# alexandre01/deepsvg

Measured on NVIDIA H100. Metric: icons/sec train-step (fwd+loss+bwd) hierarchical_ordered, higher is better.
Workload: dtype bf16

## Files before the change

### deepsvg_b200/csrc/attention_mma.cu

```cuda
#include "../../include/dsvg_b200.h"
#include "common.cuh"

namespace dsvg {
extern unsigned long long g_launches;

constexpr int kRow = 40;
constexpr int kTile = 32 * kRow;

struct MmaAttnArgs {
  const bf16* qkv;
  const uint8_t* valid;
  bf16* out;
  const bf16* dout;
  bf16* dqkv;
  int nseq, L, H;
  float scale;
  Dropout drop;
  int causal;
};

__device__ __forceinline__ void mma_bf16(float (&c)[4], const uint32_t (&a)[4], uint32_t b0, uint32_t b1) {
  asm volatile(
      "mma.sync.aligned.m16n8k16.row.col.f32.bf16.bf16.f32 {%0,%1,%2,%3}, {%4,%5,%6,%7}, {%8,%9}, {%0,%1,%2,%3};\n"
      : "+f"(c[0]), "+f"(c[1]), "+f"(c[2]), "+f"(c[3])
      : "r"(a[0]), "r"(a[1]), "r"(a[2]), "r"(a[3]), "r"(b0), "r"(b1));
}
__device__ __forceinline__ void ldsm_x4(uint32_t (&r)[4], uint32_t addr) {
  asm volatile("ldmatrix.sync.aligned.m8n8.x4.shared.b16 {%0,%1,%2,%3}, [%4];\n"
               : "=r"(r[0]), "=r"(r[1]), "=r"(r[2]), "=r"(r[3]) : "r"(addr));
}
__device__ __forceinline__ void ldsm_x4_t(uint32_t (&r)[4], uint32_t addr) {
  asm volatile("ldmatrix.sync.aligned.m8n8.x4.trans.shared.b16 {%0,%1,%2,%3}, [%4];\n"
               : "=r"(r[0]), "=r"(r[1]), "=r"(r[2]), "=r"(r[3]) : "r"(addr));
}
__device__ __forceinline__ uint32_t pack_bf16(float lo, float hi) {
  __nv_bfloat162 v = __floats2bfloat162_rn(lo, hi);
  return *reinterpret_cast<uint32_t*>(&v);
}
__device__ __forceinline__ uint32_t smem_addr(const void* p) { return uint32_t(__cvta_generic_to_shared(p)); }

__device__ __forceinline__ void load_a(uint32_t (&a)[4], uint32_t tile, int mt, int ks, int lane) {
  const int m = lane >> 3, r = lane & 7;
  ldsm_x4(a, tile + ((16 * mt + (m & 1) * 8 + r) * kRow + 16 * ks + (m >> 1) * 8) * 2);
}
__device__ __forceinline__ void load_a_t(uint32_t (&a)[4], uint32_t tile, int mt, int ks, int lane) {
  const int m = lane >> 3, r = lane & 7;
  ldsm_x4_t(a, tile + ((16 * ks + (m >> 1) * 8 + r) * kRow + 16 * mt + (m & 1) * 8) * 2);
}
__device__ __forceinline__ void load_b_nk(uint32_t (&b)[4], uint32_t tile, int np, int ks, int lane) {
  const int m = lane >> 3, r = lane & 7;
  ldsm_x4(b, tile + ((16 * np + (m >> 1) * 8 + r) * kRow + 16 * ks + (m & 1) * 8) * 2);
}
__device__ __forceinline__ void load_b_kn(uint32_t (&b)[4], uint32_t tile, int np, int ks, int lane) {
  const int m = lane >> 3, r = lane & 7;
  ldsm_x4_t(b, tile + ((16 * ks + (m & 1) * 8 + r) * kRow + 16 * np + (m >> 1) * 8) * 2);
}

__device__ __forceinline__ void stage_tile(bf16* dst, const bf16* src, int ld, int L, int lane) {
#pragma unroll
  for (int it = 0; it < 4; ++it) {
    const int chunk = lane + 32 * it, row = chunk >> 2, part = chunk & 3;
    uint4 v = make_uint4(0, 0, 0, 0);
    if (row < L) v = *reinterpret_cast<const uint4*>(src + size_t(row) * ld + part * 8);
    *reinterpret_cast<uint4*>(dst + row * kRow + part * 8) = v;
  }
}

__device__ __forceinline__ void softmax_rows(float (&s)[2][4][4], uint32_t key_mask, int t, int g = 0, int causal = 0) {
#pragma unroll
  for (int mt = 0; mt < 2; ++mt)
#pragma unroll
    for (int hrow = 0; hrow < 2; ++hrow) {
      float m = -INFINITY;
      const int i = 16 * mt + g + 8 * hrow;
      const uint32_t km = causal ? (key_mask & (0xFFFFFFFFu >> (31 - i))) : key_mask;
#pragma unroll
      for (int nt = 0; nt < 4; ++nt)
#pragma unroll
        for (int e = 0; e < 2; ++e) {
          const int j = 8 * nt + 2 * t + e;
          float& x = s[mt][nt][2 * hrow + e];
          if (!((km >> j) & 1u)) x = -INFINITY;
          m = fmaxf(m, x);
        }
      m = fmaxf(m, __shfl_xor_sync(0xffffffffu, m, 1));
      m = fmaxf(m, __shfl_xor_sync(0xffffffffu, m, 2));
      float sum = 0.f;
#pragma unroll
      for (int nt = 0; nt < 4; ++nt)
#pragma unroll
        for (int e = 0; e < 2; ++e) {
          float& x = s[mt][nt][2 * hrow + e];
          x = __expf(x - m);
          sum += x;
        }
      sum += __shfl_xor_sync(0xffffffffu, sum, 1);
      sum += __shfl_xor_sync(0xffffffffu, sum, 2);
      const float inv = 1.f / sum;
#pragma unroll
      for (int nt = 0; nt < 4; ++nt)
#pragma unroll
        for (int e = 0; e < 2; ++e) s[mt][nt][2 * hrow + e] *= inv;
    }
}

__device__ __forceinline__ void dropout_tile(float (&mult)[2][4][4], const Dropout& d, unsigned long long pair, int g,
                                             int t) {
#pragma unroll
  for (int mt = 0; mt < 2; ++mt)
#pragma unroll
    for (int hrow = 0; hrow < 2; ++hrow) {
      const int i = 16 * mt + g + 8 * hrow;
      const unsigned long long quad = ((pair * 32 + i) * 4 + t) * 2;
      const uint32_t hk = drop_hikey(d, quad), q0 = uint32_t(quad);
#pragma unroll
      for (int hq = 0; hq < 2; ++hq) {
        const uint32_t s1 = drop_stage1(q0 + hq, hk);
        const uint32_t a = drop_fin_a(s1), b = drop_fin_b(s1);
        mult[mt][2 * hq][2 * hrow] = drop_keep_lo(a, d.thr16) ? d.scale : 0.f;
        mult[mt][2 * hq][2 * hrow + 1] = drop_keep_hi(a, d.thr16) ? d.scale : 0.f;
        mult[mt][2 * hq + 1][2 * hrow] = drop_keep_lo(b, d.thr16) ? d.scale : 0.f;
        mult[mt][2 * hq + 1][2 * hrow + 1] = drop_keep_hi(b, d.thr16) ? d.scale : 0.f;
      }
    }
}

__device__ __forceinline__ uint32_t key_mask_of(const uint8_t* valid, size_t row0, int L, int lane) {
  bool ok = lane < L;
  if (ok && valid != nullptr) ok = valid[row0 + lane] != 0;
  return __ballot_sync(0xffffffffu, ok);
}

__device__ __forceinline__ void qk_scores(float (&s)[2][4][4], uint32_t q_tile, uint32_t k_tile, int lane) {
#pragma unroll
  for (int mt = 0; mt < 2; ++mt)
#pragma unroll
    for (int nt = 0; nt < 4; ++nt)
#pragma unroll
      for (int e = 0; e < 4; ++e) s[mt][nt][e] = 0.f;
#pragma unroll
  for (int ks = 0; ks < 2; ++ks) {
    uint32_t a[2][4];
    load_a(a[0], q_tile, 0, ks, lane);
    load_a(a[1], q_tile, 1, ks, lane);
#pragma unroll
    for (int np = 0; np < 2; ++np) {
      uint32_t b[4];
      load_b_nk(b, k_tile, np, ks, lane);
#pragma unroll
      for (int mt = 0; mt < 2; ++mt) {
        mma_bf16(s[mt][2 * np], a[mt], b[0], b[1]);
        mma_bf16(s[mt][2 * np + 1], a[mt], b[2], b[3]);
      }
    }
  }
}

__device__ __forceinline__ void c_to_a(uint32_t (&a)[4], const float (&c)[2][4][4], int mt, int ks) {
  a[0] = pack_bf16(c[mt][2 * ks][0], c[mt][2 * ks][1]);
  a[1] = pack_bf16(c[mt][2 * ks][2], c[mt][2 * ks][3]);
  a[2] = pack_bf16(c[mt][2 * ks + 1][0], c[mt][2 * ks + 1][1]);
  a[3] = pack_bf16(c[mt][2 * ks + 1][2], c[mt][2 * ks + 1][3]);
}
__device__ __forceinline__ void mul_regs_kn(float (&o)[2][4][4], const float (&p)[2][4][4], uint32_t y_tile, int lane) {
#pragma unroll
  for (int mt = 0; mt < 2; ++mt)
#pragma unroll
    for (int nt = 0; nt < 4; ++nt)
#pragma unroll
      for (int e = 0; e < 4; ++e) o[mt][nt][e] = 0.f;
#pragma unroll
  for (int ks = 0; ks < 2; ++ks) {
    uint32_t a[2][4];
    c_to_a(a[0], p, 0, ks);
    c_to_a(a[1], p, 1, ks);
#pragma unroll
    for (int np = 0; np < 2; ++np) {
      uint32_t b[4];
      load_b_kn(b, y_tile, np, ks, lane);
#pragma unroll
      for (int mt = 0; mt < 2; ++mt) {
        mma_bf16(o[mt][2 * np], a[mt], b[0], b[1]);
        mma_bf16(o[mt][2 * np + 1], a[mt], b[2], b[3]);
      }
    }
  }
}
__device__ __forceinline__ void mul_t_kn(float (&o)[2][4][4], uint32_t z_tile, uint32_t y_tile, int lane) {
#pragma unroll
  for (int mt = 0; mt < 2; ++mt)
#pragma unroll
    for (int nt = 0; nt < 4; ++nt)
#pragma unroll
      for (int e = 0; e < 4; ++e) o[mt][nt][e] = 0.f;
#pragma unroll
  for (int ks = 0; ks < 2; ++ks) {
    uint32_t a[2][4];
    load_a_t(a[0], z_tile, 0, ks, lane);
    load_a_t(a[1], z_tile, 1, ks, lane);
#pragma unroll
    for (int np = 0; np < 2; ++np) {
      uint32_t b[4];
      load_b_kn(b, y_tile, np, ks, lane);
#pragma unroll
      for (int mt = 0; mt < 2; ++mt) {
        mma_bf16(o[mt][2 * np], a[mt], b[0], b[1]);
        mma_bf16(o[mt][2 * np + 1], a[mt], b[2], b[3]);
      }
    }
  }
}
__device__ __forceinline__ void store_c_global(bf16* dst, int ld, int L, const float (&c)[2][4][4], float mul, int g,
                                               int t) {
#pragma unroll
  for (int mt = 0; mt < 2; ++mt)
#pragma unroll
    for (int hrow = 0; hrow < 2; ++hrow) {
      const int i = 16 * mt + g + 8 * hrow;
      if (i < L) {
#pragma unroll
        for (int nt = 0; nt < 4; ++nt)
          *reinterpret_cast<uint32_t*>(dst + size_t(i) * ld + 8 * nt + 2 * t) =
              pack_bf16(c[mt][nt][2 * hrow] * mul, c[mt][nt][2 * hrow + 1] * mul);
      }
    }
}
__device__ __forceinline__ void store_c_smem(bf16* tile, const float (&c)[2][4][4], int g, int t) {
#pragma unroll
  for (int mt = 0; mt < 2; ++mt)
#pragma unroll
    for (int hrow = 0; hrow < 2; ++hrow) {
      const int i = 16 * mt + g + 8 * hrow;
#pragma unroll
      for (int nt = 0; nt < 4; ++nt)
        *reinterpret_cast<uint32_t*>(tile + i * kRow + 8 * nt + 2 * t) = pack_bf16(c[mt][nt][2 * hrow], c[mt][nt][2 * hrow + 1]);
    }
}

constexpr int kMmaWarps = 4;

__global__ void __launch_bounds__(kMmaWarps * 32) attn_mma_fwd_kernel(MmaAttnArgs a) {
  pdl_launch_dependents();
  pdl_wait();
  drop_resolve(a.drop);
  __shared__ __align__(16) bf16 sm[kMmaWarps][3 * kTile];
  const int wib = threadIdx.x >> 5, lane = threadIdx.x & 31, g = lane >> 2, t = lane & 3;
  const int L = a.L, d = a.H * 32, ld = 3 * d;
  bf16* Qs = sm[wib];
  bf16* Ks = Qs + kTile;
  bf16* Vs = Ks + kTile;
  const uint32_t q_t = smem_addr(Qs), k_t = smem_addr(Ks), v_t = smem_addr(Vs);
  const long long npairs = (long long)a.nseq * a.H;
  for (long long pair = (long long)blockIdx.x * kMmaWarps + wib; pair < npairs; pair += (long long)gridDim.x * kMmaWarps) {
    const int seq = int(pair / a.H), h = int(pair % a.H);
    const size_t row0 = size_t(seq) * L;
    const bf16* base = a.qkv + row0 * ld + h * 32;
    stage_tile(Qs, base, ld, L, lane);
    stage_tile(Ks, base + d, ld, L, lane);
    stage_tile(Vs, base + 2 * d, ld, L, lane);
    const uint32_t kmask = key_mask_of(a.valid, row0, L, lane);
    __syncwarp();
    float s[2][4][4];
    qk_scores(s, q_t, k_t, lane);
    softmax_rows(s, kmask, t, g, a.causal);
    if (a.drop.p > 0.f) {
      float mult[2][4][4];
      dropout_tile(mult, a.drop, (unsigned long long)pair, g, t);
#pragma unroll
      for (int mt = 0; mt < 2; ++mt)
#pragma unroll
        for (int nt = 0; nt < 4; ++nt)
#pragma unroll
          for (int e = 0; e < 4; ++e) s[mt][nt][e] *= mult[mt][nt][e];
    }
    float o[2][4][4];
    mul_regs_kn(o, s, v_t, lane);
    store_c_global(a.out + row0 * d + h * 32, d, L, o, 1.f, g, t);
    __syncwarp();
  }
}

__global__ void __launch_bounds__(kMmaWarps * 32) attn_mma_bwd_kernel(MmaAttnArgs a) {
  pdl_launch_dependents();
  pdl_wait();
  drop_resolve(a.drop);
  extern __shared__ __align__(16) bf16 sm_dyn[];
  const int wib = threadIdx.x >> 5, lane = threadIdx.x & 31, g = lane >> 2, t = lane & 3;
  const int L = a.L, d = a.H * 32, ld = 3 * d;
  bf16* Qs = sm_dyn + wib * 6 * kTile;
  bf16* Ks = Qs + kTile;
  bf16* Vs = Ks + kTile;
  bf16* Gs = Vs + kTile;
  bf16* Ps = Gs + kTile;
  bf16* Ds = Ps + kTile;
  const uint32_t q_t = smem_addr(Qs), k_t = smem_addr(Ks), v_t = smem_addr(Vs), g_t = smem_addr(Gs),
                 p_t = smem_addr(Ps), d_t = smem_addr(Ds);
  const long long npairs = (long long)a.nseq * a.H;
  for (long long pair = (long long)blockIdx.x * kMmaWarps + wib; pair < npairs; pair += (long long)gridDim.x * kMmaWarps) {
    const int seq = int(pair / a.H), h = int(pair % a.H);
    const size_t row0 = size_t(seq) * L;
    const bf16* base = a.qkv + row0 * ld + h * 32;
    stage_tile(Qs, base, ld, L, lane);
    stage_tile(Ks, base + d, ld, L, lane);
    stage_tile(Vs, base + 2 * d, ld, L, lane);
    stage_tile(Gs, a.dout + row0 * d + h * 32, d, L, lane);
    const uint32_t kmask = key_mask_of(a.valid, row0, L, lane);
    __syncwarp();
    float p[2][4][4], dp[2][4][4];
    qk_scores(p, q_t, k_t, lane);
    softmax_rows(p, kmask, t, g, a.causal);
    qk_scores(dp, g_t, v_t, lane);
    if (a.drop.p > 0.f) {
      float mult[2][4][4];
      dropout_tile(mult, a.drop, (unsigned long long)pair, g, t);
#pragma unroll
      for (int mt = 0; mt < 2; ++mt)
#pragma unroll
        for (int nt = 0; nt < 4; ++nt)
#pragma unroll
          for (int e = 0; e < 4; ++e) {
            dp[mt][nt][e] *= mult[mt][nt][e];
            mult[mt][nt][e] *= p[mt][nt][e];
          }
      store_c_smem(Ps, mult, g, t);
    } else {
      store_c_smem(Ps, p, g, t);
    }
#pragma unroll
    for (int mt = 0; mt < 2; ++mt)
#pragma unroll
      for (int hrow = 0; hrow < 2; ++hrow) {
        float delta = 0.f;
#pragma unroll
        for (int nt = 0; nt < 4; ++nt)
#pragma unroll
          for (int e = 0; e < 2; ++e) delta = fmaf(dp[mt][nt][2 * hrow + e], p[mt][nt][2 * hrow + e], delta);
        delta += __shfl_xor_sync(0xffffffffu, delta, 1);
        delta += __shfl_xor_sync(0xffffffffu, delta, 2);
#pragma unroll
        for (int nt = 0; nt < 4; ++nt)
#pragma unroll
          for (int e = 0; e < 2; ++e)
            dp[mt][nt][2 * hrow + e] = p[mt][nt][2 * hrow + e] * (dp[mt][nt][2 * hrow + e] - delta);
      }
    store_c_smem(Ds, dp, g, t);
    __syncwarp();
    float o[2][4][4];
    bf16* dbase = a.dqkv + row0 * ld + h * 32;
    mul_regs_kn(o, dp, k_t, lane);
    store_c_global(dbase, ld, L, o, a.scale, g, t);
    mul_t_kn(o, d_t, q_t, lane);
    store_c_global(dbase + d, ld, L, o, 1.f, g, t);
    mul_t_kn(o, p_t, g_t, lane);
    store_c_global(dbase + 2 * d, ld, L, o, 1.f, g, t);
    __syncwarp();
  }
}


constexpr int kX3Warps = 2;
constexpr int kX3FwdTiles = 6;
constexpr int kX3BwdTiles = 10;

__device__ __forceinline__ uint32_t pack_lo(float a, float b, uint32_t hi) {
  const __nv_bfloat162 h = *reinterpret_cast<const __nv_bfloat162*>(&hi);
  const float2 hf = __bfloat1622float2(h);
  return pack_bf16(a - hf.x, b - hf.y);
}
#define DSVG_MMA3(acc, ah, al, bh, bl, i, j)   \
  mma_bf16(acc, al, bh[i], bh[j]);              \
  mma_bf16(acc, ah, bl[i], bl[j]);              \
  mma_bf16(acc, ah, bh[i], bh[j])
__device__ __forceinline__ void qk_scores_x3(float (&s)[2][4][4], uint32_t x_t, uint32_t y_t, int lane) {
#pragma unroll
  for (int mt = 0; mt < 2; ++mt)
#pragma unroll
    for (int nt = 0; nt < 4; ++nt)
#pragma unroll
      for (int e = 0; e < 4; ++e) s[mt][nt][e] = 0.f;
#pragma unroll
  for (int ks = 0; ks < 2; ++ks) {
    uint32_t ah[2][4], al[2][4];
    load_a(ah[0], x_t, 0, ks, lane);
    load_a(ah[1], x_t, 1, ks, lane);
    load_a(al[0], x_t + kTile * 2, 0, ks, lane);
    load_a(al[1], x_t + kTile * 2, 1, ks, lane);
#pragma unroll
    for (int np = 0; np < 2; ++np) {
      uint32_t bh[4], bl[4];
      load_b_nk(bh, y_t, np, ks, lane);
      load_b_nk(bl, y_t + kTile * 2, np, ks, lane);
#pragma unroll
      for (int mt = 0; mt < 2; ++mt) {
        DSVG_MMA3(s[mt][2 * np], ah[mt], al[mt], bh, bl, 0, 1);
        DSVG_MMA3(s[mt][2 * np + 1], ah[mt], al[mt], bh, bl, 2, 3);
      }
    }
  }
}
__device__ __forceinline__ void c_to_a_x3(uint32_t (&ah)[4], uint32_t (&al)[4], const float (&c)[2][4][4], int mt, int ks) {
  c_to_a(ah, c, mt, ks);
  al[0] = pack_lo(c[mt][2 * ks][0], c[mt][2 * ks][1], ah[0]);
  al[1] = pack_lo(c[mt][2 * ks][2], c[mt][2 * ks][3], ah[1]);
  al[2] = pack_lo(c[mt][2 * ks + 1][0], c[mt][2 * ks + 1][1], ah[2]);
  al[3] = pack_lo(c[mt][2 * ks + 1][2], c[mt][2 * ks + 1][3], ah[3]);
}
__device__ __forceinline__ void mul_regs_kn_x3(float (&o)[2][4][4], const float (&p)[2][4][4], uint32_t y_t, int lane) {
#pragma unroll
  for (int mt = 0; mt < 2; ++mt)
#pragma unroll
    for (int nt = 0; nt < 4; ++nt)
// ... 166 lines not shown
    softmax_rows(p, kmask, t, g, a.causal);
    qk_scores_x3(dp, g_t, v_t, lane);
    __syncwarp();
    if (a.drop.p > 0.f) {
      float mult[2][4][4];
      dropout_tile(mult, a.drop, (unsigned long long)pair, g, t);
#pragma unroll
      for (int mt = 0; mt < 2; ++mt)
#pragma unroll
        for (int nt = 0; nt < 4; ++nt)
#pragma unroll
          for (int e = 0; e < 4; ++e) {
            dp[mt][nt][e] *= mult[mt][nt][e];
            mult[mt][nt][e] *= p[mt][nt][e];
          }
      store_c_smem_x3(Ps, mult, g, t);
    } else {
      store_c_smem_x3(Ps, p, g, t);
    }
#pragma unroll
    for (int mt = 0; mt < 2; ++mt)
#pragma unroll
      for (int hrow = 0; hrow < 2; ++hrow) {
        float delta = 0.f;
#pragma unroll
        for (int nt = 0; nt < 4; ++nt)
#pragma unroll
          for (int e = 0; e < 2; ++e) delta = fmaf(dp[mt][nt][2 * hrow + e], p[mt][nt][2 * hrow + e], delta);
        delta += __shfl_xor_sync(0xffffffffu, delta, 1);
        delta += __shfl_xor_sync(0xffffffffu, delta, 2);
#pragma unroll
        for (int nt = 0; nt < 4; ++nt)
#pragma unroll
          for (int e = 0; e < 2; ++e)
            dp[mt][nt][2 * hrow + e] = p[mt][nt][2 * hrow + e] * (dp[mt][nt][2 * hrow + e] - delta);
      }
    store_c_smem_x3(Ds, dp, g, t);
    __syncwarp();
    float o[2][4][4];
    bf16* dbase = a.dqkv + row0 * ld + h * 32;
    mul_regs_kn_x3(o, dp, k_t, lane);
    store_c_global_x3(dbase, x.dqkv_lo, ld, L, o, a.scale, g, t);
    mul_t_kn_x3(o, d_t, q_t, lane);
    store_c_global_x3(dbase + d, x.dqkv_lo, ld, L, o, 1.f, g, t);
    mul_t_kn_x3(o, p_t, g_t, lane);
    store_c_global_x3(dbase + 2 * d, x.dqkv_lo, ld, L, o, 1.f, g, t);
    __syncwarp();
  }
}

}
using namespace dsvg;

static long long mma_grid_cap(bool bwd) {
  static long long cap[2] = {0, 0};
  if (cap[bwd] == 0) {
    int n = 0;
    if (bwd) cudaOccupancyMaxActiveBlocksPerMultiprocessor(&n, dsvg::attn_mma_bwd_kernel, dsvg::kMmaWarps * 32, size_t(dsvg::kMmaWarps * 6 * dsvg::kTile * 2));
    else cudaOccupancyMaxActiveBlocksPerMultiprocessor(&n, dsvg::attn_mma_fwd_kernel, dsvg::kMmaWarps * 32, 0);
    cap[bwd] = 132LL * (n > 0 ? n : 8);
  }
  return cap[bwd];
}

int dsvg_attn_mma_fwd(const bf16* qkv, const uint8_t* valid, bf16* out, int nseq, int L, int H, Dropout drop, int causal,
                      cudaStream_t st) {
  MmaAttnArgs a{};
  a.qkv = qkv; a.valid = valid; a.out = out; a.nseq = nseq; a.L = L; a.H = H; a.scale = 1.f; a.drop = drop;
  a.causal = causal;
  long long blocks = ((long long)nseq * H + kMmaWarps - 1) / kMmaWarps;
  if (blocks > mma_grid_cap(false)) blocks = mma_grid_cap(false);
  DSVG_CUDA(launch_k(attn_mma_fwd_kernel, dim3(int(blocks)), dim3(kMmaWarps * 32), 0, st, a));
  ++g_launches;
  return 0;
}
int dsvg_attn_mma_bwd(const bf16* qkv, const uint8_t* valid, const bf16* dout, bf16* dqkv, int nseq, int L, int H,
                      float q_scale, Dropout drop, int causal, cudaStream_t st) {
  MmaAttnArgs a{};
  a.qkv = qkv; a.valid = valid; a.dout = dout; a.dqkv = dqkv; a.nseq = nseq; a.L = L; a.H = H; a.scale = q_scale;
  a.drop = drop; a.causal = causal;
  constexpr int smem = kMmaWarps * 6 * kTile * 2;
  static bool configured[kMaxDevices] = {};
  if (first_use_on_device(configured)) {
    DSVG_CUDA(cudaFuncSetAttribute(attn_mma_bwd_kernel, cudaFuncAttributeMaxDynamicSharedMemorySize, smem));
  }
  long long blocks = ((long long)nseq * H + kMmaWarps - 1) / kMmaWarps;
  if (blocks > mma_grid_cap(true)) blocks = mma_grid_cap(true);
  DSVG_CUDA(launch_k(attn_mma_bwd_kernel, dim3(int(blocks)), dim3(kMmaWarps * 32), size_t(smem), st, a));
  ++g_launches;
  return 0;
}

int dsvg_attn_x3(bool bwd, const bf16* qkv, size_t qkv_lo, const uint8_t* valid, bf16* out, size_t out_lo, const bf16* dout,
                 size_t dout_lo, bf16* dqkv, size_t dqkv_lo, int nseq, int L, int H, float q_scale, Dropout drop, int causal,
                 cudaStream_t st) {
  X3AttnArgs x{};
  MmaAttnArgs& a = x.m;
  a.qkv = qkv; a.valid = valid; a.out = out; a.dout = dout; a.dqkv = dqkv; a.nseq = nseq; a.L = L; a.H = H;
  a.scale = q_scale; a.drop = drop; a.causal = causal;
  x.qkv_lo = qkv_lo; x.out_lo = out_lo; x.dout_lo = dout_lo; x.dqkv_lo = dqkv_lo;
  const int smem = kX3Warps * (bwd ? kX3BwdTiles : kX3FwdTiles) * kTile * 2;
  static bool configured[kMaxDevices] = {};
  static long long cap[2] = {0, 0};
  if (first_use_on_device(configured)) {
    DSVG_CUDA(cudaFuncSetAttribute(attn_x3_fwd_kernel, cudaFuncAttributeMaxDynamicSharedMemorySize,
                                   kX3Warps * kX3FwdTiles * kTile * 2));
    DSVG_CUDA(cudaFuncSetAttribute(attn_x3_bwd_kernel, cudaFuncAttributeMaxDynamicSharedMemorySize,
                                   kX3Warps * kX3BwdTiles * kTile * 2));
  }
  if (cap[bwd] == 0) {
    int n = 0;
    if (bwd) cudaOccupancyMaxActiveBlocksPerMultiprocessor(&n, attn_x3_bwd_kernel, kX3Warps * 32, size_t(smem));
    else cudaOccupancyMaxActiveBlocksPerMultiprocessor(&n, attn_x3_fwd_kernel, kX3Warps * 32, size_t(smem));
    cap[bwd] = 132LL * (n > 0 ? n : 4);
  }
  long long blocks = ((long long)nseq * H + kX3Warps - 1) / kX3Warps;
  if (blocks > cap[bwd]) blocks = cap[bwd];
  if (bwd) DSVG_CUDA(launch_k(attn_x3_bwd_kernel, dim3(int(blocks)), dim3(kX3Warps * 32), size_t(smem), st, x));
  else DSVG_CUDA(launch_k(attn_x3_fwd_kernel, dim3(int(blocks)), dim3(kX3Warps * 32), size_t(smem), st, x));
  ++g_launches;
  return 0;
}

namespace dsvg {

__device__ __forceinline__ void g_load_a(uint32_t (&a)[4], uint32_t tile, int row0, int k0, int st, int lane) {
  const int m = lane >> 3, r = lane & 7;
  ldsm_x4(a, tile + ((row0 + (m & 1) * 8 + r) * st + k0 + (m >> 1) * 8) * 2);
}
__device__ __forceinline__ void g_load_a_t(uint32_t (&a)[4], uint32_t tile, int m0, int k0, int st, int lane) {
  const int m = lane >> 3, r = lane & 7;
  ldsm_x4_t(a, tile + ((k0 + (m >> 1) * 8 + r) * st + m0 + (m & 1) * 8) * 2);
}
__device__ __forceinline__ void g_load_b_nk(uint32_t (&b)[4], uint32_t tile, int n0, int k0, int st, int lane) {
  const int m = lane >> 3, r = lane & 7;
  ldsm_x4(b, tile + ((n0 + (m >> 1) * 8 + r) * st + k0 + (m & 1) * 8) * 2);
}
__device__ __forceinline__ void g_load_b_kn(uint32_t (&b)[4], uint32_t tile, int n0, int k0, int st, int lane) {
  const int m = lane >> 3, r = lane & 7;
  ldsm_x4_t(b, tile + ((k0 + (m & 1) * 8 + r) * st + n0 + (m >> 1) * 8) * 2);
}

template <int HD, int NT>
// ... 697 lines not shown
```

### deepsvg_b200/csrc/ptx.cuh

```cuda
#pragma once
#include <cstdint>
#include <cuda.h>
#include <cuda_runtime.h>

namespace dsvg {

__device__ __forceinline__ uint32_t smem_u32(const void* p) {
  return static_cast<uint32_t>(__cvta_generic_to_shared(p));
}

__device__ __forceinline__ bool elect_one() {
  uint32_t pred = 0;
  asm volatile(
      "{\n\t.reg .pred P;\n\t"
      "elect.sync _|P, 0xffffffff;\n\t"
      "selp.u32 %0, 1, 0, P;\n\t}\n"
      : "=r"(pred));
  return pred != 0;
}

__device__ __forceinline__ void mbar_init(uint64_t* bar, uint32_t count) {
  asm volatile("mbarrier.init.shared::cta.b64 [%0], %1;" ::"r"(smem_u32(bar)), "r"(count) : "memory");
}
__device__ __forceinline__ void fence_barrier_init() {
  asm volatile("fence.mbarrier_init.release.cluster;" ::: "memory");
}
__device__ __forceinline__ void mbar_arrive_expect_tx(uint64_t* bar, uint32_t bytes) {
  asm volatile("mbarrier.arrive.expect_tx.shared::cta.b64 _, [%0], %1;" ::"r"(smem_u32(bar)), "r"(bytes)
               : "memory");
}
__device__ __forceinline__ void mbar_arrive(uint64_t* bar) {
  asm volatile("mbarrier.arrive.shared::cta.b64 _, [%0];" ::"r"(smem_u32(bar)) : "memory");
}
__device__ __forceinline__ bool mbar_try_wait(uint64_t* bar, uint32_t parity) {
  uint32_t ok;
  asm volatile(
      "{\n\t.reg .pred P;\n\t"
      "mbarrier.try_wait.parity.shared::cta.b64 P, [%1], %2;\n\t"
      "selp.u32 %0, 1, 0, P;\n\t}\n"
      : "=r"(ok)
      : "r"(smem_u32(bar)), "r"(parity)
      : "memory");
  return ok != 0;
}
__device__ __forceinline__ void mbar_wait(uint64_t* bar, uint32_t parity) {
  uint32_t spins = 0;
  while (!mbar_try_wait(bar, parity)) {
    if (++spins > (1u << 26)) __trap();
  }
}

__device__ __forceinline__ void fence_proxy_async_smem() {
  asm volatile("fence.proxy.async.shared::cta;" ::: "memory");
}

__device__ __forceinline__ void tma_prefetch_desc(const CUtensorMap* m) {
  asm volatile("prefetch.tensormap [%0];" ::"l"(reinterpret_cast<uint64_t>(m)) : "memory");
}
__device__ __forceinline__ void tma_load_2d(void* smem_dst, const CUtensorMap* m, uint64_t* bar, int c0,
                                            int c1) {
  asm volatile(
      "cp.async.bulk.tensor.2d.shared::cluster.global.mbarrier::complete_tx::bytes [%0], [%1, {%3, %4}], [%2];"
      ::"r"(smem_u32(smem_dst)),
      "l"(reinterpret_cast<uint64_t>(m)), "r"(smem_u32(bar)), "r"(c0), "r"(c1)
      : "memory");
}

__device__ __forceinline__ void tma_store_2d(const CUtensorMap* m, const void* smem_src, int c0, int c1) {
  asm volatile("cp.async.bulk.tensor.2d.global.shared::cta.bulk_group [%0, {%2, %3}], [%1];" ::"l"(
                   reinterpret_cast<uint64_t>(m)),
               "r"(smem_u32(smem_src)), "r"(c0), "r"(c1)
               : "memory");
}
__device__ __forceinline__ void tma_store_commit() { asm volatile("cp.async.bulk.commit_group;" ::: "memory"); }
__device__ __forceinline__ void tma_store_wait_read() { asm volatile("cp.async.bulk.wait_group.read 0;" ::: "memory"); }
template <int N>
__device__ __forceinline__ void tma_store_wait_read_n() {
  asm volatile("cp.async.bulk.wait_group.read %0;" ::"n"(N) : "memory");
}
__device__ __forceinline__ void tma_store_wait_all() { asm volatile("cp.async.bulk.wait_group 0;" ::: "memory"); }
__device__ __forceinline__ void named_bar_sync(int id, int nthreads) {
  asm volatile("bar.sync %0, %1;" ::"r"(id), "r"(nthreads) : "memory");
}

template <int R>
__device__ __forceinline__ void setmaxnreg_dec() { asm volatile("setmaxnreg.dec.sync.aligned.u32 %0;" ::"n"(R)); }
template <int R>
__device__ __forceinline__ void setmaxnreg_inc() { asm volatile("setmaxnreg.inc.sync.aligned.u32 %0;" ::"n"(R)); }

__device__ __forceinline__ void wgmma_fence() { asm volatile("wgmma.fence.sync.aligned;" ::: "memory"); }
__device__ __forceinline__ void wgmma_commit() { asm volatile("wgmma.commit_group.sync.aligned;" ::: "memory"); }
template <int N>
__device__ __forceinline__ void wgmma_wait() {
  asm volatile("wgmma.wait_group.sync.aligned %0;" ::"n"(N) : "memory");
}
template <int R>
__device__ __forceinline__ void wgmma_fence_regs(float (&d)[R]) {
#pragma unroll
  for (int i = 0; i < R; ++i) asm volatile("" : "+f"(d[i])::"memory");
}

__device__ __forceinline__ void wgmma_m64n32_kk(float (&d)[16], uint64_t adesc, uint64_t bdesc) {
  asm volatile(
      "{\n\t.reg .pred p;\n\tsetp.ne.b32 p, %18, 0;\n\t"
      "wgmma.mma_async.sync.aligned.m64n32k16.f32.bf16.bf16 "
      "{%0, %1, %2, %3, %4, %5, %6, %7, %8, %9, %10, %11, %12, %13, %14, %15}, %16, %17, p, 1, 1, 0, 0;\n\t}\n"
      : "+f"(d[0]), "+f"(d[1]), "+f"(d[2]), "+f"(d[3]), "+f"(d[4]), "+f"(d[5]), "+f"(d[6]), "+f"(d[7]), "+f"(d[8]),
        "+f"(d[9]), "+f"(d[10]), "+f"(d[11]), "+f"(d[12]), "+f"(d[13]), "+f"(d[14]), "+f"(d[15])
      : "l"(adesc), "l"(bdesc), "r"(1));
}
__device__ __forceinline__ void wgmma_m64n256_kk(float (&d)[128], uint64_t adesc, uint64_t bdesc) {
  asm volatile(
      "{\n\t.reg .pred p;\n\tsetp.ne.b32 p, %130, 0;\n\t"
      "wgmma.mma_async.sync.aligned.m64n256k16.f32.bf16.bf16 {"
      "%0, %1, %2, %3, %4, %5, %6, %7, %8, %9, %10, %11, %12, %13, %14, %15, "
      "%16, %17, %18, %19, %20, %21, %22, %23, %24, %25, %26, %27, %28, %29, %30, %31, "
      "%32, %33, %34, %35, %36, %37, %38, %39, %40, %41, %42, %43, %44, %45, %46, %47, "
      "%48, %49, %50, %51, %52, %53, %54, %55, %56, %57, %58, %59, %60, %61, %62, %63, "
      "%64, %65, %66, %67, %68, %69, %70, %71, %72, %73, %74, %75, %76, %77, %78, %79, "
      "%80, %81, %82, %83, %84, %85, %86, %87, %88, %89, %90, %91, %92, %93, %94, %95, "
      "%96, %97, %98, %99, %100, %101, %102, %103, %104, %105, %106, %107, %108, %109, %110, %111, "
      "%112, %113, %114, %115, %116, %117, %118, %119, %120, %121, %122, %123, %124, %125, %126, %127"
      "}, %128, %129, p, 1, 1, 0, 0;\n\t}\n"
      : "+f"(d[0]), "+f"(d[1]), "+f"(d[2]), "+f"(d[3]), "+f"(d[4]), "+f"(d[5]), "+f"(d[6]), "+f"(d[7]),
// ... 70 lines not shown
```

Measured before the change: 21460.

## Stream whole-sequence attention tiles via bulk async copies with producer warp pipeline

Replaces the per-(sequence,head) warp kernels with a warp-specialized design. A producer warp bulk-loads whole sequence rows (all heads of QKV, plus dout for the backward pass) into double-buffered shared memory with mbarriers. Consumer warps each take one head and write their results back in place in shared memory, and the producer then bulk-stores full contiguous rows. This removes the strided per-head global loads and scattered global stores and overlaps copies with MMA work. The cost is a large shared-memory footprint that limits occupancy, plus new constraints on L, H and pointer alignment.

After: 22520 (median of 6 runs). 1.05x the previous value.

```diff
diff --git a/deepsvg_b200/csrc/attention_mma.cu b/deepsvg_b200/csrc/attention_mma.cu
--- a/deepsvg_b200/csrc/attention_mma.cu
+++ b/deepsvg_b200/csrc/attention_mma.cu
@@ -1,5 +1,6 @@
 #include "../../include/dsvg_b200.h"
 #include "common.cuh"
+#include "ptx.cuh"
 
 namespace dsvg {
 extern unsigned long long g_launches;
@@ -17,6 +18,7 @@
   float scale;
   Dropout drop;
   int causal;
+  int stages;
 };
 
 __device__ __forceinline__ void mma_bf16(float (&c)[4], const uint32_t (&a)[4], uint32_t b0, uint32_t b1) {
@@ -39,21 +41,21 @@
 }
 __device__ __forceinline__ uint32_t smem_addr(const void* p) { return uint32_t(__cvta_generic_to_shared(p)); }
 
-__device__ __forceinline__ void load_a(uint32_t (&a)[4], uint32_t tile, int mt, int ks, int lane) {
+__device__ __forceinline__ void load_a(uint32_t (&a)[4], uint32_t tile, int mt, int ks, int lane, int st = kRow) {
   const int m = lane >> 3, r = lane & 7;
-  ldsm_x4(a, tile + ((16 * mt + (m & 1) * 8 + r) * kRow + 16 * ks + (m >> 1) * 8) * 2);
-}
-__device__ __forceinline__ void load_a_t(uint32_t (&a)[4], uint32_t tile, int mt, int ks, int lane) {
+  ldsm_x4(a, tile + ((16 * mt + (m & 1) * 8 + r) * st + 16 * ks + (m >> 1) * 8) * 2);
+}
+__device__ __forceinline__ void load_a_t(uint32_t (&a)[4], uint32_t tile, int mt, int ks, int lane, int st = kRow) {
   const int m = lane >> 3, r = lane & 7;
-  ldsm_x4_t(a, tile + ((16 * ks + (m >> 1) * 8 + r) * kRow + 16 * mt + (m & 1) * 8) * 2);
-}
-__device__ __forceinline__ void load_b_nk(uint32_t (&b)[4], uint32_t tile, int np, int ks, int lane) {
+  ldsm_x4_t(a, tile + ((16 * ks + (m >> 1) * 8 + r) * st + 16 * mt + (m & 1) * 8) * 2);
+}
+__device__ __forceinline__ void load_b_nk(uint32_t (&b)[4], uint32_t tile, int np, int ks, int lane, int st = kRow) {
   const int m = lane >> 3, r = lane & 7;
-  ldsm_x4(b, tile + ((16 * np + (m >> 1) * 8 + r) * kRow + 16 * ks + (m & 1) * 8) * 2);
-}
-__device__ __forceinline__ void load_b_kn(uint32_t (&b)[4], uint32_t tile, int np, int ks, int lane) {
+  ldsm_x4(b, tile + ((16 * np + (m >> 1) * 8 + r) * st + 16 * ks + (m & 1) * 8) * 2);
+}
+__device__ __forceinline__ void load_b_kn(uint32_t (&b)[4], uint32_t tile, int np, int ks, int lane, int st = kRow) {
   const int m = lane >> 3, r = lane & 7;
-  ldsm_x4_t(b, tile + ((16 * ks + (m & 1) * 8 + r) * kRow + 16 * np + (m >> 1) * 8) * 2);
+  ldsm_x4_t(b, tile + ((16 * ks + (m & 1) * 8 + r) * st + 16 * np + (m >> 1) * 8) * 2);
 }
 
 __device__ __forceinline__ void stage_tile(bf16* dst, const bf16* src, int ld, int L, int lane) {
@@ -131,7 +133,8 @@
   return __ballot_sync(0xffffffffu, ok);
 }
 
-__device__ __forceinline__ void qk_scores(float (&s)[2][4][4], uint32_t q_tile, uint32_t k_tile, int lane) {
+__device__ __forceinline__ void qk_scores(float (&s)[2][4][4], uint32_t q_tile, uint32_t k_tile, int lane, int qs = kRow,
+                                          int kst = kRow) {
 #pragma unroll
   for (int mt = 0; mt < 2; ++mt)
 #pragma unroll
@@ -141,12 +144,12 @@
 #pragma unroll
   for (int ks = 0; ks < 2; ++ks) {
     uint32_t a[2][4];
-    load_a(a[0], q_tile, 0, ks, lane);
-    load_a(a[1], q_tile, 1, ks, lane);
+    load_a(a[0], q_tile, 0, ks, lane, qs);
+    load_a(a[1], q_tile, 1, ks, lane, qs);
 #pragma unroll
     for (int np = 0; np < 2; ++np) {
       uint32_t b[4];
-      load_b_nk(b, k_tile, np, ks, lane);
+      load_b_nk(b, k_tile, np, ks, lane, kst);
 #pragma unroll
       for (int mt = 0; mt < 2; ++mt) {
         mma_bf16(s[mt][2 * np], a[mt], b[0], b[1]);
@@ -162,7 +165,8 @@
   a[2] = pack_bf16(c[mt][2 * ks + 1][0], c[mt][2 * ks + 1][1]);
   a[3] = pack_bf16(c[mt][2 * ks + 1][2], c[mt][2 * ks + 1][3]);
 }
-__device__ __forceinline__ void mul_regs_kn(float (&o)[2][4][4], const float (&p)[2][4][4], uint32_t y_tile, int lane) {
+__device__ __forceinline__ void mul_regs_kn(float (&o)[2][4][4], const float (&p)[2][4][4], uint32_t y_tile, int lane,
+                                            int ys = kRow) {
 #pragma unroll
   for (int mt = 0; mt < 2; ++mt)
 #pragma unroll
@@ -177,7 +181,7 @@
 #pragma unroll
     for (int np = 0; np < 2; ++np) {
       uint32_t b[4];
-      load_b_kn(b, y_tile, np, ks, lane);
+      load_b_kn(b, y_tile, np, ks, lane, ys);
 #pragma unroll
       for (int mt = 0; mt < 2; ++mt) {
         mma_bf16(o[mt][2 * np], a[mt], b[0], b[1]);
@@ -186,7 +190,8 @@
     }
   }
 }
-__device__ __forceinline__ void mul_t_kn(float (&o)[2][4][4], uint32_t z_tile, uint32_t y_tile, int lane) {
+__device__ __forceinline__ void mul_t_kn(float (&o)[2][4][4], uint32_t z_tile, uint32_t y_tile, int lane, int zs = kRow,
+                                         int ys = kRow) {
 #pragma unroll
   for (int mt = 0; mt < 2; ++mt)
 #pragma unroll
@@ -196,12 +201,12 @@
 #pragma unroll
   for (int ks = 0; ks < 2; ++ks) {
     uint32_t a[2][4];
-    load_a_t(a[0], z_tile, 0, ks, lane);
-    load_a_t(a[1], z_tile, 1, ks, lane);
+    load_a_t(a[0], z_tile, 0, ks, lane, zs);
+    load_a_t(a[1], z_tile, 1, ks, lane, zs);
 #pragma unroll
     for (int np = 0; np < 2; ++np) {
       uint32_t b[4];
-      load_b_kn(b, y_tile, np, ks, lane);
+      load_b_kn(b, y_tile, np, ks, lane, ys);
 #pragma unroll
       for (int mt = 0; mt < 2; ++mt) {
         mma_bf16(o[mt][2 * np], a[mt], b[0], b[1]);
@@ -210,8 +215,7 @@
     }
   }
 }
-__device__ __forceinline__ void store_c_global(bf16* dst, int ld, int L, const float (&c)[2][4][4], float mul, int g,
-                                               int t) {
+__device__ __forceinline__ void store_c_rows(bf16* tile, int st, int L, const float (&c)[2][4][4], float mul, int g, int t) {
 #pragma unroll
   for (int mt = 0; mt < 2; ++mt)
 #pragma unroll
@@ -220,7 +224,7 @@
       if (i < L) {
 #pragma unroll
         for (int nt = 0; nt < 4; ++nt)
-          *reinterpret_cast<uint32_t*>(dst + size_t(i) * ld + 8 * nt + 2 * t) =
+          *reinterpret_cast<uint32_t*>(tile + i * st + 8 * nt + 2 * t) =
               pack_bf16(c[mt][nt][2 * hrow] * mul, c[mt][nt][2 * hrow + 1] * mul);
       }
     }
@@ -237,126 +241,203 @@
     }
 }
 
-constexpr int kMmaWarps = 4;
-
-__global__ void __launch_bounds__(kMmaWarps * 32) attn_mma_fwd_kernel(MmaAttnArgs a) {
+constexpr int kStreamWarps = 8;
+constexpr int kStreamRows = 32;
+constexpr int kStreamMaxStages = 2;
+constexpr int kStreamBarBytes = 64;
+constexpr int kStreamSmemMax = 227 * 1024;
+
+__host__ __device__ constexpr int stream_qkv_stride(int H) { return 96 * H + 8; }
+__host__ __device__ constexpr int stream_dout_stride(int H) { return 32 * H + 8; }
+__host__ __device__ constexpr int stream_stage_elems(int H, bool bwd) {
+  return kStreamRows * (stream_qkv_stride(H) + (bwd ? stream_dout_stride(H) : 0));
+}
+
+__device__ __forceinline__ void stream_init(unsigned char* smem, int stage_bytes, int stages, int consumers) {
+  uint4* z = reinterpret_cast<uint4*>(smem + kStreamBarBytes);
+  for (int i = threadIdx.x; i < stages * stage_bytes / 16; i += blockDim.x) z[i] = make_uint4(0, 0, 0, 0);
+  fence_proxy_async_smem();
+  uint64_t* bars = reinterpret_cast<uint64_t*>(smem);
+  if (threadIdx.x == 0) {
+    for (int s = 0; s < stages; ++s) {
+      mbar_init(&bars[s], 1);
+      mbar_init(&bars[kStreamMaxStages + s], consumers);
+    }
+    fence_barrier_init();
+  }
+  __syncthreads();
+}
+
+__device__ __forceinline__ void stream_producer(unsigned char* smem, int stage_elems, int stages, const MmaAttnArgs& a,
+                                                bool bwd, int lane) {
+  uint64_t* full = reinterpret_cast<uint64_t*>(smem);
+  uint64_t* empty = full + kStreamMaxStages;
+  bf16* stage0 = reinterpret_cast<bf16*>(smem + kStreamBarBytes);
+  const int L = a.L, d = a.H * 32, rs = stream_qkv_stride(a.H), rd = stream_dout_stride(a.H);
+  const int n = (a.nseq - int(blockIdx.x) + int(gridDim.x) - 1) / int(gridDim.x);
+  const uint32_t row_in = uint32_t(3 * d * 2 + (bwd ? d * 2 : 0));
+  const int out_cols = bwd ? 3 * d : d;
+  bf16* dst = bwd ? a.dqkv : a.out;
+  for (int k = 0; k < n + stages; ++k) {
+    const int s = k % stages;
+    bf16* qkv_st = stage0 + size_t(s) * stage_elems;
+    if (k >= stages) {
+      mbar_wait(&empty[s], uint32_t((k / stages - 1) & 1));
+      const size_t row0 = size_t(int(blockIdx.x) + (k - stages) * int(gridDim.x)) * L;
+      if (lane < L) bulk_store(dst + (row0 + lane) * out_cols, qkv_st + lane * rs, uint32_t(out_cols * 2));
+      tma_store_commit();
+    }
+    if (k < n) {
+      if (k >= stages) tma_store_wait_read();
+      const size_t row0 = size_t(int(blockIdx.x) + k * int(gridDim.x)) * L;
+      if (lane == 0) mbar_arrive_expect_tx(&full[s], uint32_t(L) * row_in);
+      __syncwarp();
+      if (lane < L) {
+        bulk_load(qkv_st + lane * rs, a.qkv + (row0 + lane) * (3 * d), uint32_t(3 * d * 2), &full[s]);
+        if (bwd)
+          bulk_load(qkv_st + kStreamRows * rs + lane * rd, a.dout + (row0 + lane) * d, uint32_t(d * 2), &full[s]);
+      }
+    }
+  }
+  tma_store_wait_all();
+}
+
+__global__ void __launch_bounds__((kStreamWarps + 1) * 32, 2) attn_mma_fwd_kernel(MmaAttnArgs a) {
   pdl_launch_dependents();
+  extern __shared__ __align__(128) unsigned char smem[];
+  const int W = int(blockDim.x >> 5) - 1, warp = threadIdx.x >> 5, lane = threadIdx.x & 31, g = lane >> 2, t = lane & 3;
+  const int L = a.L, H = a.H, d = H * 32, rs = stream_qkv_stride(H), stages = a.stages;
+  const int stage_elems = stream_stage_elems(H, false);
+  stream_init(smem, stage_elems * 2, stages, W * 32);
   pdl_wait();
+  if (warp == W) {
+    stream_producer(smem, stage_elems, stages, a, false, lane);
+    return;
+  }
   drop_resolve(a.drop);
-  __shared__ __align__(16) bf16 sm[kMmaWarps][3 * kTile];
-  const int wib = threadIdx.x >> 5, lane = threadIdx.x & 31, g = lane >> 2, t = lane & 3;
-  const int L = a.L, d = a.H * 32, ld = 3 * d;
-  bf16* Qs = sm[wib];
-  bf16* Ks = Qs + kTile;
-  bf16* Vs = Ks + kTile;
-  const uint32_t q_t = smem_addr(Qs), k_t = smem_addr(Ks), v_t = smem_addr(Vs);
-  const long long npairs = (long long)a.nseq * a.H;
-  for (long long pair = (long long)blockIdx.x * kMmaWarps + wib; pair < npairs; pair += (long long)gridDim.x * kMmaWarps) {
-    const int seq = int(pair / a.H), h = int(pair % a.H);
+  uint64_t* full = reinterpret_cast<uint64_t*>(smem);
+  uint64_t* empty = full + kStreamMaxStages;
+  bf16* stage0 = reinterpret_cast<bf16*>(smem + kStreamBarBytes);
+  const int n = (a.nseq - int(blockIdx.x) + int(gridDim.x) - 1) / int(gridDim.x);
+  for (int k = 0; k < n; ++k) {
+    const int s = k % stages, seq = int(blockIdx.x) + k * int(gridDim.x);
     const size_t row0 = size_t(seq) * L;
-    const bf16* base = a.qkv + row0 * ld + h * 32;
-    stage_tile(Qs, base, ld, L, lane);
-    stage_tile(Ks, base + d, ld, L, lane);
-    stage_tile(Vs, base + 2 * d, ld, L, lane);
     const uint32_t kmask = key_mask_of(a.valid, row0, L, lane);
-    __syncwarp();
-    float s[2][4][4];
-    qk_scores(s, q_t, k_t, lane);
-    softmax_rows(s, kmask, t, g, a.causal);
-    if (a.drop.p > 0.f) {
-      float mult[2][4][4];
-      dropout_tile(mult, a.drop, (unsigned long long)pair, g, t);
+    bf16* st = stage0 + size_t(s) * stage_elems;
+    mbar_wait(&full[s], uint32_t((k / stages) & 1));
+    for (int h = warp; h < H; h += W) {
+      bf16* Qs = st + h * 32;
+      const uint32_t q_t = smem_addr(Qs), k_t = smem_addr(Qs + d), v_t = smem_addr(Qs + 2 * d);
+      const long long pair = (long long)seq * H + h;
+      float sc[2][4][4];
+      qk_scores(sc, q_t, k_t, lane, rs, rs);
+      softmax_rows(sc, kmask, t, g, a.causal);
+      if (a.drop.p > 0.f) {
+        float mult[2][4][4];
+        dropout_tile(mult, a.drop, (unsigned long long)pair, g, t);
+#pragma unroll
+        for (int mt = 0; mt < 2; ++mt)
+#pragma unroll
+          for (int nt = 0; nt < 4; ++nt)
+#pragma unroll
+            for (int e = 0; e < 4; ++e) sc[mt][nt][e] *= mult[mt][nt][e];
+      }
+      float o[2][4][4];
+      mul_regs_kn(o, sc, v_t, lane, rs);
+      __syncwarp();
+      store_c_rows(Qs, rs, L, o, 1.f, g, t);
+    }
+    fence_proxy_async_smem();
+    mbar_arrive(&empty[s]);
+  }
+}
+
+__global__ void __launch_bounds__((kStreamWarps + 1) * 32, 1) attn_mma_bwd_kernel(MmaAttnArgs a) {
+  pdl_launch_dependents();
+  extern __shared__ __align__(128) unsigned char smem[];
+  const int W = int(blockDim.x >> 5) - 1, warp = threadIdx.x >> 5, lane = threadIdx.x & 31, g = lane >> 2, t = lane & 3;
+  const int L = a.L, H = a.H, d = H * 32, rs = stream_qkv_stride(H), rd = stream_dout_stride(H), stages = a.stages;
+  const int stage_elems = stream_stage_elems(H, true);
+  stream_init(smem, stage_elems * 2, stages, W * 32);
+  pdl_wait();
+  if (warp == W) {
+    stream_producer(smem, stage_elems, stages, a, true, lane);
+    return;
+  }
+  drop_resolve(a.drop);
+  uint64_t* full = reinterpret_cast<uint64_t*>(smem);
+  uint64_t* empty = full + kStreamMaxStages;
+  bf16* stage0 = reinterpret_cast<bf16*>(smem + kStreamBarBytes);
+  bf16* Ps = stage0 + size_t(stages) * stage_elems + warp * 2 * kTile;
+  bf16* Ds = Ps + kTile;
+  const uint32_t p_t = smem_addr(Ps), d_t = smem_addr(Ds);
+  const int n = (a.nseq - int(blockIdx.x) + int(gridDim.x) - 1) / int(gridDim.x);
+  for (int k = 0; k < n; ++k) {
+    const int s = k % stages, seq = int(blockIdx.x) + k * int(gridDim.x);
+    const size_t row0 = size_t(seq) * L;
+    const uint32_t kmask = key_mask_of(a.valid, row0, L, lane);
+    bf16* st = stage0 + size_t(s) * stage_elems;
+    mbar_wait(&full[s], uint32_t((k / stages) & 1));
+    for (int h = warp; h < H; h += W) {
+      bf16* Qs = st + h * 32;
+      bf16* Ks = Qs + d;
+      bf16* Vs = Qs + 2 * d;
+      bf16* Gs = st + kStreamRows * rs + h * 32;
+      const uint32_t q_t = smem_addr(Qs), k_t = smem_addr(Ks), v_t = smem_addr(Vs), g_t = smem_addr(Gs);
+      const long long pair = (long long)seq * H + h;
+      float p[2][4][4], dp[2][4][4];
+      qk_scores(p, q_t, k_t, lane, rs, rs);
+      softmax_rows(p, kmask, t, g, a.causal);
+      qk_scores(dp, g_t, v_t, lane, rd, rs);
+      if (a.drop.p > 0.f) {
+        float mult[2][4][4];
+        dropout_tile(mult, a.drop, (unsigned long long)pair, g, t);
+#pragma unroll
+        for (int mt = 0; mt < 2; ++mt)
+#pragma unroll
+          for (int nt = 0; nt < 4; ++nt)
+#pragma unroll
+            for (int e = 0; e < 4; ++e) {
+              dp[mt][nt][e] *= mult[mt][nt][e];
+              mult[mt][nt][e] *= p[mt][nt][e];
+            }
+        store_c_smem(Ps, mult, g, t);
+      } else {
+        store_c_smem(Ps, p, g, t);
+      }
 #pragma unroll
       for (int mt = 0; mt < 2; ++mt)
 #pragma unroll
-        for (int nt = 0; nt < 4; ++nt)
-#pragma unroll
-          for (int e = 0; e < 4; ++e) s[mt][nt][e] *= mult[mt][nt][e];
-    }
-    float o[2][4][4];
-    mul_regs_kn(o, s, v_t, lane);
-    store_c_global(a.out + row0 * d + h * 32, d, L, o, 1.f, g, t);
-    __syncwarp();
-  }
-}
-
-__global__ void __launch_bounds__(kMmaWarps * 32) attn_mma_bwd_kernel(MmaAttnArgs a) {
-  pdl_launch_dependents();
-  pdl_wait();
-  drop_resolve(a.drop);
-  extern __shared__ __align__(16) bf16 sm_dyn[];
-  const int wib = threadIdx.x >> 5, lane = threadIdx.x & 31, g = lane >> 2, t = lane & 3;
-  const int L = a.L, d = a.H * 32, ld = 3 * d;
-  bf16* Qs = sm_dyn + wib * 6 * kTile;
-  bf16* Ks = Qs + kTile;
-  bf16* Vs = Ks + kTile;
-  bf16* Gs = Vs + kTile;
-  bf16* Ps = Gs + kTile;
-  bf16* Ds = Ps + kTile;
-  const uint32_t q_t = smem_addr(Qs), k_t = smem_addr(Ks), v_t = smem_addr(Vs), g_t = smem_addr(Gs),
-                 p_t = smem_addr(Ps), d_t = smem_addr(Ds);
-  const long long npairs = (long long)a.nseq * a.H;
-  for (long long pair = (long long)blockIdx.x * kMmaWarps + wib; pair < npairs; pair += (long long)gridDim.x * kMmaWarps) {
-    const int seq = int(pair / a.H), h = int(pair % a.H);
-    const size_t row0 = size_t(seq) * L;
-    const bf16* base = a.qkv + row0 * ld + h * 32;
-    stage_tile(Qs, base, ld, L, lane);
-    stage_tile(Ks, base + d, ld, L, lane);
-    stage_tile(Vs, base + 2 * d, ld, L, lane);
-    stage_tile(Gs, a.dout + row0 * d + h * 32, d, L, lane);
-    const uint32_t kmask = key_mask_of(a.valid, row0, L, lane);
-    __syncwarp();
-    float p[2][4][4], dp[2][4][4];
-    qk_scores(p, q_t, k_t, lane);
-    softmax_rows(p, kmask, t, g, a.causal);
-    qk_scores(dp, g_t, v_t, lane);
-    if (a.drop.p > 0.f) {
-      float mult[2][4][4];
-      dropout_tile(mult, a.drop, (unsigned long long)pair, g, t);
-#pragma unroll
-      for (int mt = 0; mt < 2; ++mt)
-#pragma unroll
-        for (int nt = 0; nt < 4; ++nt)
-#pragma unroll
-          for (int e = 0; e < 4; ++e) {
-            dp[mt][nt][e] *= mult[mt][nt][e];
-            mult[mt][nt][e] *= p[mt][nt][e];
-          }
-      store_c_smem(Ps, mult, g, t);
-    } else {
-      store_c_smem(Ps, p, g, t);
-    }
-#pragma unroll
-    for (int mt = 0; mt < 2; ++mt)
-#pragma unroll
-      for (int hrow = 0; hrow < 2; ++hrow) {
-        float delta = 0.f;
-#pragma unroll
-        for (int nt = 0; nt < 4; ++nt)
-#pragma unroll
-          for (int e = 0; e < 2; ++e) delta = fmaf(dp[mt][nt][2 * hrow + e], p[mt][nt][2 * hrow + e], delta);
-        delta += __shfl_xor_sync(0xffffffffu, delta, 1);
-        delta += __shfl_xor_sync(0xffffffffu, delta, 2);
-#pragma unroll
-        for (int nt = 0; nt < 4; ++nt)
-#pragma unroll
-          for (int e = 0; e < 2; ++e)
-            dp[mt][nt][2 * hrow + e] = p[mt][nt][2 * hrow + e] * (dp[mt][nt][2 * hrow + e] - delta);
-      }
-    store_c_smem(Ds, dp, g, t);
-    __syncwarp();
-    float o[2][4][4];
-    bf16* dbase = a.dqkv + row0 * ld + h * 32;
-    mul_regs_kn(o, dp, k_t, lane);
-    store_c_global(dbase, ld, L, o, a.scale, g, t);
-    mul_t_kn(o, d_t, q_t, lane);
-    store_c_global(dbase + d, ld, L, o, 1.f, g, t);
-    mul_t_kn(o, p_t, g_t, lane);
-    store_c_global(dbase + 2 * d, ld, L, o, 1.f, g, t);
-    __syncwarp();
-  }
-}
-
+        for (int hrow = 0; hrow < 2; ++hrow) {
+          float delta = 0.f;
+#pragma unroll
+          for (int nt = 0; nt < 4; ++nt)
+#pragma unroll
+            for (int e = 0; e < 2; ++e) delta = fmaf(dp[mt][nt][2 * hrow + e], p[mt][nt][2 * hrow + e], delta);
+          delta += __shfl_xor_sync(0xffffffffu, delta, 1);
+          delta += __shfl_xor_sync(0xffffffffu, delta, 2);
+#pragma unroll
+          for (int nt = 0; nt < 4; ++nt)
+#pragma unroll
+            for (int e = 0; e < 2; ++e)
+              dp[mt][nt][2 * hrow + e] = p[mt][nt][2 * hrow + e] * (dp[mt][nt][2 * hrow + e] - delta);
+        }
+      store_c_smem(Ds, dp, g, t);
+      __syncwarp();
+      float oq[2][4][4], ok[2][4][4];
+      mul_regs_kn(oq, dp, k_t, lane, rs);
+      mul_t_kn(ok, d_t, q_t, lane, kRow, rs);
+      __syncwarp();
+      store_c_rows(Qs, rs, L, oq, a.scale, g, t);
+      store_c_rows(Ks, rs, L, ok, 1.f, g, t);
+      mul_t_kn(oq, p_t, g_t, lane, kRow, rd);
+      store_c_rows(Vs, rs, L, oq, 1.f, g, t);
+      __syncwarp();
+    }
+    fence_proxy_async_smem();
+    mbar_arrive(&empty[s]);
+  }
+}
 
 constexpr int kX3Warps = 2;
 constexpr int kX3FwdTiles = 6;
@@ -629,15 +710,32 @@
 }
 using namespace dsvg;
 
-static long long mma_grid_cap(bool bwd) {
-  static long long cap[2] = {0, 0};
-  if (cap[bwd] == 0) {
-    int n = 0;
-    if (bwd) cudaOccupancyMaxActiveBlocksPerMultiprocessor(&n, dsvg::attn_mma_bwd_kernel, dsvg::kMmaWarps * 32, size_t(dsvg::kMmaWarps * 6 * dsvg::kTile * 2));
-    else cudaOccupancyMaxActiveBlocksPerMultiprocessor(&n, dsvg::attn_mma_fwd_kernel, dsvg::kMmaWarps * 32, 0);
-    cap[bwd] = 132LL * (n > 0 ? n : 8);
-  }
-  return cap[bwd];
+static int launch_stream(bool bwd, MmaAttnArgs& a, cudaStream_t st) {
+  DSVG_CHECK(a.L >= 1 && a.L <= kStreamRows, "attn_mma: L = %d outside 1..%d", a.L, kStreamRows);
+  const uintptr_t align = reinterpret_cast<uintptr_t>(a.qkv) | reinterpret_cast<uintptr_t>(a.out) |
+                          reinterpret_cast<uintptr_t>(a.dout) | reinterpret_cast<uintptr_t>(a.dqkv);
+  DSVG_CHECK((align & 15) == 0, "attn_mma: qkv / dout / outputs must be 16-byte aligned for the bulk copies");
+  const int W = a.H < kStreamWarps ? a.H : kStreamWarps;
+  const long long stage = 2LL * stream_stage_elems(a.H, bwd);
+  const long long fixed = kStreamBarBytes + (bwd ? 2LL * W * 2 * kTile : 0);
+  a.stages = fixed + 2 * stage <= kStreamSmemMax ? 2 : 1;
+  const long long smem = fixed + a.stages * stage;
+  DSVG_CHECK(smem <= kStreamSmemMax, "attn_mma: H = %d heads need %lld bytes of shared memory per sequence (max %d)", a.H,
+             smem, kStreamSmemMax);
+  auto kern = bwd ? attn_mma_bwd_kernel : attn_mma_fwd_kernel;
+  static bool configured[2][kMaxDevices] = {};
+  if (first_use_on_device(configured[bwd]))
+    DSVG_CUDA(cudaFuncSetAttribute(kern, cudaFuncAttributeMaxDynamicSharedMemorySize, kStreamSmemMax));
+  int dev = 0, sms = 0, per_sm = 0;
+  DSVG_CUDA(cudaGetDevice(&dev));
+  DSVG_CUDA(cudaDeviceGetAttribute(&sms, cudaDevAttrMultiProcessorCount, dev));
+  DSVG_CUDA(cudaOccupancyMaxActiveBlocksPerMultiprocessor(&per_sm, kern, (W + 1) * 32, size_t(smem)));
+  DSVG_CHECK(per_sm > 0, "attn_mma: %lld bytes of shared memory per CTA do not fit", smem);
+  long long blocks = (long long)sms * per_sm;
+  if (blocks > a.nseq) blocks = a.nseq;
+  DSVG_CUDA(launch_k(kern, dim3(int(blocks)), dim3((W + 1) * 32), size_t(smem), st, a));
+  ++g_launches;
+  return 0;
 }
 
 int dsvg_attn_mma_fwd(const bf16* qkv, const uint8_t* valid, bf16* out, int nseq, int L, int H, Dropout drop, int causal,
@@ -645,27 +743,14 @@
   MmaAttnArgs a{};
   a.qkv = qkv; a.valid = valid; a.out = out; a.nseq = nseq; a.L = L; a.H = H; a.scale = 1.f; a.drop = drop;
   a.causal = causal;
-  long long blocks = ((long long)nseq * H + kMmaWarps - 1) / kMmaWarps;
-  if (blocks > mma_grid_cap(false)) blocks = mma_grid_cap(false);
-  DSVG_CUDA(launch_k(attn_mma_fwd_kernel, dim3(int(blocks)), dim3(kMmaWarps * 32), 0, st, a));
-  ++g_launches;
-  return 0;
+  return launch_stream(false, a, st);
 }
 int dsvg_attn_mma_bwd(const bf16* qkv, const uint8_t* valid, const bf16* dout, bf16* dqkv, int nseq, int L, int H,
                       float q_scale, Dropout drop, int causal, cudaStream_t st) {
   MmaAttnArgs a{};
   a.qkv = qkv; a.valid = valid; a.dout = dout; a.dqkv = dqkv; a.nseq = nseq; a.L = L; a.H = H; a.scale = q_scale;
   a.drop = drop; a.causal = causal;
-  constexpr int smem = kMmaWarps * 6 * kTile * 2;
-  static bool configured[kMaxDevices] = {};
-  if (first_use_on_device(configured)) {
-    DSVG_CUDA(cudaFuncSetAttribute(attn_mma_bwd_kernel, cudaFuncAttributeMaxDynamicSharedMemorySize, smem));
-  }
-  long long blocks = ((long long)nseq * H + kMmaWarps - 1) / kMmaWarps;
-  if (blocks > mma_grid_cap(true)) blocks = mma_grid_cap(true);
-  DSVG_CUDA(launch_k(attn_mma_bwd_kernel, dim3(int(blocks)), dim3(kMmaWarps * 32), size_t(smem), st, a));
-  ++g_launches;
-  return 0;
+  return launch_stream(true, a, st);
 }
 
 int dsvg_attn_x3(bool bwd, const bf16* qkv, size_t qkv_lo, const uint8_t* valid, bf16* out, size_t out_lo, const bf16* dout,
diff --git a/deepsvg_b200/csrc/ptx.cuh b/deepsvg_b200/csrc/ptx.cuh
--- a/deepsvg_b200/csrc/ptx.cuh
+++ b/deepsvg_b200/csrc/ptx.cuh
@@ -70,6 +70,16 @@
   asm volatile("cp.async.bulk.tensor.2d.global.shared::cta.bulk_group [%0, {%2, %3}], [%1];" ::"l"(
                    reinterpret_cast<uint64_t>(m)),
                "r"(smem_u32(smem_src)), "r"(c0), "r"(c1)
+               : "memory");
+}
+__device__ __forceinline__ void bulk_load(void* smem_dst, const void* src, uint32_t bytes, uint64_t* bar) {
+  asm volatile("cp.async.bulk.shared::cluster.global.mbarrier::complete_tx::bytes [%0], [%1], %2, [%3];"
+               ::"r"(smem_u32(smem_dst)), "l"(reinterpret_cast<uint64_t>(src)), "r"(bytes), "r"(smem_u32(bar))
+               : "memory");
+}
+__device__ __forceinline__ void bulk_store(void* dst, const void* smem_src, uint32_t bytes) {
+  asm volatile("cp.async.bulk.global.shared::cta.bulk_group [%0], [%1], %2;"
+               ::"l"(reinterpret_cast<uint64_t>(dst)), "r"(smem_u32(smem_src)), "r"(bytes)
                : "memory");
 }
 __device__ __forceinline__ void tma_store_commit() { asm volatile("cp.async.bulk.commit_group;" ::: "memory"); }
```
